# Adamtaranto/mimeo

Hardware: AMD Instinct MI355X
Metric: Gbp-aligned/sec (mimeo self, 1 Gbp genome, --minIdt 80 --minLen 100 --minCov 3) (higher is better)
Workload: dtype int32

## Files before the change

mimeo_amd/csrc/k34_fused.hip:

```cpp
#include <cstdio>
#include <algorithm>
#include <cstdlib>
#include <mutex>
#include <type_traits>

#include "k4_device.h"

namespace mimeo {

constexpr uint32_t TCH = 64;
constexpr uint32_t DQ = 192;
constexpr uint32_t CARE10 = 0x1A997u;
constexpr unsigned long long HEAVY_HITS = 262144;
constexpr unsigned long long PART_HITS = 131072;
constexpr uint32_t HEAVY_GRID = 2048;

struct FusedArgs {
    const FusedUnit *units;
    ExtQueues q;
    HeavyPlan plan;
    int xdrop, hspthresh, transitions;
    uint32_t dbg;
};

struct Bound2 {
    int32_t up, lomax, ub;
    bool stop;
};
template <int W>
__device__ __forceinline__ void bound_block2(Bound2 &B, uint32_t v, uint32_t n, int32_t &lo, int xdrop) {
    const int32_t pv = __popc(v), pn = __popc(n);
    B.ub = max(B.ub, B.up + 100 * W - 100 * pn);
    B.up += 100 * W - 131 * pn - 83 * pv;
    lo += 91 * W - 122 * pn - 94 * pv;
    B.stop = B.stop || (B.up + xdrop < B.lomax);
    B.lomax = max(B.lomax, lo);
}

template <uint32_t CARE, bool TV>
__device__ __forceinline__ uint32_t seed_starts32(uint32_t n0, uint32_t n1, uint32_t d0, uint32_t d1, int transitions) {
    uint32_t ones = 0, twos = 0, tv = 0;
#pragma unroll
    for (int c = 0; c < SEED_LEN; c++) {
        if (!((CARE >> c) & 1u)) continue;
        const uint32_t v = __builtin_amdgcn_alignbit(n1, n0, 13 + c);
        twos |= ones & v;
        ones |= v;
        if (TV) tv |= __builtin_amdgcn_alignbit(d1, d0, 13 + c);
    }
    return ~(transitions ? (twos | tv) : ones);
}

__device__ __forceinline__ bool pair_needs_walk(const uint4 t0, const uint4 t1, const uint4 t2, const uint4 q0, const uint4 q1,
                                                const uint4 q2, int xdrop, int hspthresh, int transitions) {
    const uint32_t dl0 = t0.x ^ q0.x, dl1 = t0.y ^ q0.y, dl2 = t0.z ^ q0.z, dl3 = t0.w ^ q0.w, dl4 = t1.x ^ q1.x, dl5 = t1.y ^ q1.y;
    const uint32_t n0 = dl0 | (t1.z ^ q1.z), n1 = dl1 | (t1.w ^ q1.w), n2 = dl2 | (t2.x ^ q2.x), n3 = dl3 | (t2.y ^ q2.y),
                   n4 = dl4 | (t2.z ^ q2.z), n5 = dl5 | (t2.w ^ q2.w);
    const uint32_t h0 = seed_starts32<CARE10, false>(n2, n3, 0u, 0u, transitions);
    const uint32_t h1 = seed_starts32<CARE10, false>(n1, n2, 0u, 0u, transitions);
    const uint32_t h2 = seed_starts32<CARE10, false>(n0, n1, 0u, 0u, transitions);
    Bound2 L{0, 0, 0, false}, R{0, 0, 0, false};
    int32_t llo = 0, rlo = 0;
    uint32_t veto;
    constexpr uint32_t M24 = 0xFFFFFFu;
    veto = h0 >> 8;
    bound_block2<24>(L, dl3 >> 8, n3 >> 8, llo, xdrop);
    veto |= L.stop ? 0u : ((h0 & 0xFFu) | (h1 >> 16));
    bound_block2<24>(L, __builtin_amdgcn_alignbit(dl3, dl2, 16) & M24, __builtin_amdgcn_alignbit(n3, n2, 16) & M24, llo, xdrop);
    veto |= L.stop ? 0u : ((h1 & 0xFFFFu) | (h2 >> 24));
    bound_block2<24>(L, __builtin_amdgcn_alignbit(dl2, dl1, 24) & M24, __builtin_amdgcn_alignbit(n2, n1, 24) & M24, llo, xdrop);
    veto |= L.stop ? 0u : (h2 & M24);
    bound_block2<24>(L, dl1 & M24, n1 & M24, llo, xdrop);
    bound_block2<24>(R, dl4 & M24, n4 & M24, rlo, xdrop);
    bound_block2<24>(R, __builtin_amdgcn_alignbit(dl5, dl4, 24) & M24, __builtin_amdgcn_alignbit(n5, n4, 24) & M24, rlo, xdrop);
    bound_block2<16>(R, dl5 >> 16, n5 >> 16, rlo, xdrop);
    return !(L.stop && R.stop && L.ub + R.ub < hspthresh && veto == 0);
}

__device__ __forceinline__ bool run_interior(const uint4 t0, const uint4 t1, const uint4 t2, const uint4 q0, const uint4 q1, const uint4 q2,
                                             int transitions) {
    const uint32_t dl3 = t0.w ^ q0.w, dl4 = t1.x ^ q1.x;
    const uint32_t n3 = dl3 | (t2.y ^ q2.y), n4 = dl4 | (t2.z ^ q2.z);
    bool all = true;
#pragma unroll
    for (int k = 0; k < 3; k++) {
        const int off = k == 0 ? 11 : (k == 1 ? 12 : 14);
        const uint32_t wn = __builtin_amdgcn_alignbit(n4, n3, off) & CARE19, wd = __builtin_amdgcn_alignbit(dl4, dl3, off) & CARE19;
        all = all && (transitions ? (wd == 0u && __popc(wn) <= 1) : (wn == 0u));
    }
    return all;
}

constexpr uint32_t DENSE_MIN = 48;
__device__ __forceinline__ uint4 readlane4(const uint4 v, int lane) {
    return make_uint4((uint32_t)__builtin_amdgcn_readlane((int)v.x, lane), (uint32_t)__builtin_amdgcn_readlane((int)v.y, lane),
                      (uint32_t)__builtin_amdgcn_readlane((int)v.z, lane), (uint32_t)__builtin_amdgcn_readlane((int)v.w, lane));
}
__device__ __forceinline__ uint4 bperm4(uint32_t src_lane, const uint4 v) {
    const int a = (int)(src_lane << 2);
    return make_uint4((uint32_t)__builtin_amdgcn_ds_bpermute(a, (int)v.x), (uint32_t)__builtin_amdgcn_ds_bpermute(a, (int)v.y),
                      (uint32_t)__builtin_amdgcn_ds_bpermute(a, (int)v.z), (uint32_t)__builtin_amdgcn_ds_bpermute(a, (int)v.w));
}

template <int THREADS, uint32_t QSEG, bool HEAVY>
struct FusedCfg {
    static constexpr int WAVES = THREADS / 64;
    static constexpr size_t OFF_BYTES = ((TILE_WORDS + 1) * 2 + 15) / 16 * 16;
    static constexpr size_t SMEM = OFF_BYTES + (size_t)QSEG * 48 + (size_t)WAVES * DQ * 4 + (size_t)WAVES * 64 * 8 + QSEG + 16;
};

template <int THREADS, uint32_t QSEG, bool HEAVY>
__global__ __launch_bounds__(THREADS, 4) void k34_scan_extend(FusedArgs A) {
    using Cfg = FusedCfg<THREADS, QSEG, HEAVY>;
    using qoff_t = uint16_t;
    constexpr int WAVES = THREADS / 64;
    static_assert((size_t)QSEG * 48 >= 2 * (TILE_WORDS + 4) * 4, "the count prologue stages both offset arrays in the frame area");
    extern __shared__ __attribute__((aligned(16))) uint8_t smem[];
    qoff_t *sQ = reinterpret_cast<qoff_t *>(smem);
    uint4 *sQF = reinterpret_cast<uint4 *>(smem + Cfg::OFF_BYTES);
    uint32_t *sD_all = reinterpret_cast<uint32_t *>(sQF + QSEG * 3);
    uint2 *s_walk_all = reinterpret_cast<uint2 *>(sD_all + WAVES * DQ);
    uint8_t *sQN = reinterpret_cast<uint8_t *>(s_walk_all + WAVES * 64);
    unsigned long long *s_total = reinterpret_cast<unsigned long long *>(sQN + QSEG);
    __shared__ unsigned long long s_slot;

    const uint32_t lane = threadIdx.x & 63u, wv = threadIdx.x >> 6;
    const uint64_t lt_mask = (1ull << lane) - 1ull;
    uint32_t ai = HEAVY ? 0u : blockIdx.y;
    GFusedUnit U = A.units[ai];
    uint32_t part_p = 0, part_pt = 1, part_qa = 0, part_qb = 0xFFFFFFFFu, part_no = 0;
    uint32_t *sD = sD_all + wv * DQ;
    uint2 *s_walk = s_walk_all + wv * 64;
    uint32_t n_walk = 0;

    auto flush_walk = [&](uint32_t n) {
        __builtin_amdgcn_wave_barrier();
        unsigned long long b = 0;
        const uint32_t shard = (HEAVY ? blockIdx.x + part_no : blockIdx.x) & 7u;
        if (lane == 0) b = atomicAdd(&A.q.nwalk_u[(size_t)ai * 8 + shard], (unsigned long long)n);
        b = __shfl(b, 0);
        if (lane < n && b + lane < U.walk_cap) {
            uint2 e = s_walk[lane];
            e.y = U.Q.pos[e.y] & POS_MASK;
            A.q.walkq[U.walk_base + (size_t)shard * U.walk_cap + b + lane] = e;
        }
        __builtin_amdgcn_wave_barrier();
    };

    auto do_tile = [&](const uint32_t tile) {
        const gptr<uint32_t> toff = U.T.off + (size_t)tile * TILE_WORDS, qoff = U.Q.off + (size_t)tile * TILE_WORDS;
        const uint32_t t0 = toff[0], nT = toff[TILE_WORDS] - t0;
        const uint32_t q0 = qoff[0], nQ = qoff[TILE_WORDS] - q0;
        if (!nT || !nQ) return;
        if (!HEAVY) {
            uint32_t *sT = reinterpret_cast<uint32_t *>(sQF), *sQ32 = sT + TILE_WORDS + 4;
            {
                const gptr<uint4> s0 = toff.as<uint4>(), s1 = qoff.as<uint4>();
                uint4 *d0 = reinterpret_cast<uint4 *>(sT), *d1 = reinterpret_cast<uint4 *>(sQ32);
                for (uint32_t k = threadIdx.x; k < TILE_WORDS / 4; k += THREADS) { const uint4 a = s0[k], b = s1[k]; d0[k] = a; d1[k] = b; }
                if (threadIdx.x == 0) { sT[TILE_WORDS] = t0 + nT; sQ32[TILE_WORDS] = q0 + nQ; *s_total = 0ull; }
            }
            __syncthreads();
            unsigned long long cnt = 0;
            for (uint32_t w = threadIdx.x; w < TILE_WORDS; w += THREADS)
                cnt += (unsigned long long)(sT[w + 1] - sT[w]) * (sQ32[w + 1] - sQ32[w]);
            for (int o = 32; o > 0; o >>= 1) cnt += __shfl_xor(cnt, o);
            if (lane == 0 && cnt) atomicAdd(s_total, cnt);
            __syncthreads();
            if (!*s_total && A.transitions) {
                __syncthreads();
                unsigned long long c2 = 0;
                for (uint32_t w = threadIdx.x; w < TILE_WORDS; w += THREADS) {
                    const uint32_t nt = sT[w + 1] - sT[w];
                    if (nt)
                        for (int j = 0; j < SEED_WEIGHT; j++) { const uint32_t w2 = w ^ (1u << j); c2 += sQ32[w2 + 1] - sQ32[w2]; }
                }
                if (__syncthreads_or(c2 != 0) == 0) return;
            } else if (!*s_total) {
                return;
            }
            const unsigned long long tile_est = *s_total * (A.transitions ? (unsigned long long)(SEED_WEIGHT + 1) : 1ull);
            if (tile_est > HEAVY_HITS || nQ > 0xFFFFu) {
                if (threadIdx.x == 0) {
                    const size_t slot = (size_t)ai * NTILE + atomicAdd(&A.q.nheavy_u[ai], 1ull);
                    A.q.heavy[slot] = tile;
                    A.q.heavy_est[slot] = tile_est;
                }
                return;
            }
        }
        constexpr int NRO = (TILE_WORDS + THREADS) / THREADS;
        uint32_t ro[NRO];
#pragma unroll
        for (int i = 0; i < NRO; i++) {
            const uint32_t k = threadIdx.x + (uint32_t)i * THREADS;
            ro[i] = 0;
            if (k <= TILE_WORDS) ro[i] = (HEAVY ? qoff[k] : (k < TILE_WORDS ? (reinterpret_cast<const uint32_t *>(sQF) + TILE_WORDS + 4)[k] : q0 + nQ)) - q0;
        }
        bool aligned = false;
        uint32_t mid = 0;
        if (!HEAVY && nQ > QSEG) {
            mid = (uint32_t)__builtin_amdgcn_readfirstlane((int)((reinterpret_cast<const uint32_t *>(sQF) + TILE_WORDS + 4)[TILE_WORDS / 2] - q0));
            aligned = mid <= QSEG && nQ - mid <= QSEG;
        }
        const gptr<uint4> tF0 = U.T.fr + t0, tF1 = tF0 + U.T.fr_stride, tF2 = tF1 + U.T.fr_stride;
        const uint32_t nchunks = (nT + TCH - 1) / TCH;
        const uint32_t ch_first = (HEAVY ? part_p * WAVES : 0u) + wv, ch_step = (HEAVY ? part_pt : 1u) * WAVES;
        uint4 nf0 = make_uint4(0, 0, 0, 0), nf1 = nf0, nf2 = nf0;
        uint32_t npos = 0;
        if (ch_first < nchunks) {
            const uint32_t e = ch_first * TCH + lane;
            if (e < nT) { nf0 = tF0[e]; nf1 = tF1[e]; nf2 = tF2[e]; npos = U.T.pos[t0 + e]; }
        }
        unsigned long long hits_acc = 0;
        auto pair_round = [&](const bool valid, const uint4 ta, const uint4 tb, const uint4 tc, const uint32_t tpf, const uint32_t qi, const uint32_t qs) {
            const uint4 qa = sQF[qi], qb = sQF[QSEG + qi], qc = sQF[2 * QSEG + qi];
            const uint32_t qflag = sQN[qi];
            bool need = false;
            uint32_t qp = 0;
            bool live = valid;
            if (HEAVY && !(A.dbg & 16u)) {
                bool inner = false;
                if (valid && ((tpf >> 31) | qflag) == 0 && !U.Tv.svt && run_interior(ta, tb, tc, qa, qb, qc, A.transitions)) {
                    const uint32_t tp = tpf & POS_MASK;
                    inner = tp >= 2u && tp + 1u + SEED_LEN <= U.Tv.len;
                }
                live = valid && !inner;
            }
            if (__ballot(live)) {
                if (live) {
                    if (A.dbg & 1u) need = (ta.x ^ qa.x ^ tb.y ^ qb.y ^ tc.z ^ qc.z) == 0x12345u;
                    else need = ((tpf >> 31) | (qflag & 1u)) != 0 ||
                                pair_needs_walk(ta, tb, tc, qa, qb, qc, A.xdrop, A.hspthresh, A.transitions);
                    if (A.dbg & 2u) need = false;
                }
            }
            if (U.same) {
                if (valid) {
                    qp = U.Q.pos[q0 + qs + qi] & POS_MASK;
                    if ((tpf & POS_MASK) == qp) need = false;
                }
            }
            const uint64_t m = __ballot(need);
            if (m) {
                const uint32_t add = (uint32_t)__popcll(m);
                if (n_walk + add > 64u) { flush_walk(n_walk); n_walk = 0; }
                if (need) s_walk[n_walk + __popcll(m & lt_mask)] = make_uint2(tpf & POS_MASK, q0 + qs + qi);
                n_walk += add;
            }
        };
        const uint32_t q_begin = HEAVY ? part_qa : 0u, q_end = HEAVY ? min(part_qb, nQ) : nQ;
        for (uint32_t qs = q_begin, qe; qs < q_end; qs = qe) {
            qe = aligned ? (qs ? q_end : mid) : min(qs + QSEG, q_end);
            const uint32_t qn = qe - qs;
            const uint32_t half = qs ? 1u : 0u;
            __syncthreads();
#pragma unroll
            for (int i = 0; i < NRO; i++) {
                const uint32_t k = threadIdx.x + (uint32_t)i * THREADS;
                if (k <= TILE_WORDS) sQ[k] = (qoff_t)(min(max(ro[i], qs), qe) - qs);
            }
            {
                const gptr<uint4> s0 = U.Q.fr + q0 + qs, s1 = s0 + U.Q.fr_stride, s2 = s1 + U.Q.fr_stride;
                const gptr<uint32_t> sp = U.Q.pos + q0 + qs;
                for (uint32_t i = threadIdx.x; i < qn; i += THREADS) {
                    const uint4 a = s0[i], b = s1[i], c = s2[i];
                    const uint32_t pq = sp[i], pp = pq & POS_MASK;
                    sQF[i] = a;
                    sQF[QSEG + i] = b;
                    sQF[2 * QSEG + i] = c;
                    sQN[i] = (uint8_t)((pq >> 31) | ((pp >= 2u && pp + 1u + SEED_LEN <= U.Qv.len) ? 0u : 2u));
                }
            }
            __syncthreads();
            for (uint32_t ch = ch_first; ch < nchunks; ch += ch_step) {
                const uint32_t e0 = ch * TCH, ne = min(TCH, nT - e0);
                const uint4 f0 = nf0, f1 = nf1, f2 = nf2;
                const uint32_t mypos = npos;
                {
                    uint32_t nx = ch + ch_step;
                    if (nx >= nchunks) nx = (qe < q_end) ? ch_first : 0xFFFFFFFFu;
                    if (nx != 0xFFFFFFFFu && nx != ch) {
                        const uint32_t e = nx * TCH + lane;
                        if (e < nT) { nf0 = tF0[e]; nf1 = tF1[e]; nf2 = tF2[e]; npos = U.T.pos[t0 + e]; }
                    }
                }
                const bool tvalid = lane < ne;
                uint32_t w = 0, c = 0, nmask = 0, dmask = 0;
                if (tvalid) w = pext12(f2.y >> 13);
                const int nn = A.transitions ? SEED_WEIGHT + 1 : 1;
                if constexpr (!HEAVY) {
                    int jlo = 0, jhi = nn;
                    if (aligned) {
                        const uint64_t in_half = __ballot(tvalid && (w >> 11) == half), in_other = __ballot(tvalid && (w >> 11) != half);
                        if (!in_other) jhi = min(nn, SEED_WEIGHT);
                        else if (!in_half) jlo = SEED_WEIGHT;
                    }
                    jlo = __builtin_amdgcn_readfirstlane(jlo);
                    jhi = __builtin_amdgcn_readfirstlane(jhi);
                    constexpr uint32_t RING = 128;
                    static_assert(RING <= DQ, "the ring lives in the wavefront's descriptor queue");
                    const uint32_t l16 = lane << 16;
                    uint32_t head = 0, tail = 0, pend = 0;
                    uint32_t an = 0, cn = 0;
                    auto fetch = [&](const int jj) {
                        an = 0; cn = 0;
                        if (tvalid && jj < jhi) {
                            const uint32_t w2 = jj ? (w ^ (1u << (jj - 1))) : w;
                            an = sQ[w2];
                            cn = (uint32_t)sQ[w2 + 1] - an;
                        }
                    };
                    auto round = [&](const uint32_t n) {
                        __builtin_amdgcn_wave_barrier();
                        const bool valid = lane < n;
                        const uint32_t d = valid ? sD[(head + lane) & (RING - 1u)] : 0u;
                        const uint32_t owner = d >> 16, qi = d & 0xFFFFu;
                        if (!(A.dbg & 4u)) {
                            const uint4 ta = bperm4(owner, f0), tb = bperm4(owner, f1), tc = bperm4(owner, f2);
                            const uint32_t tpf = (uint32_t)__builtin_amdgcn_ds_bpermute((int)(owner << 2), (int)mypos);
                            pair_round(valid, ta, tb, tc, tpf, qi, qs);
                        }
                        __builtin_amdgcn_wave_barrier();
                        head = (head + 64u) & (RING - 1u);
                        pend -= n;
                    };
                    fetch(jlo);
#pragma unroll 1
                    for (int j = jlo; j < jhi; j++) {
                        const uint32_t ak = l16 | an, cnt = cn;
                        fetch(j + 1);
                        uint32_t k = 0;
#pragma unroll 1
                        for (uint64_t m = __ballot(cnt > 0u); m; m = __ballot(cnt > k)) {
                            if (cnt > k) {
                                const uint32_t slot = __builtin_amdgcn_mbcnt_hi((uint32_t)(m >> 32), __builtin_amdgcn_mbcnt_lo((uint32_t)m, tail));
                                sD[slot & (RING - 1u)] = ak + k;
                            }
                            const uint32_t add = (uint32_t)__popcll(m);
                            tail = (tail + add) & (RING - 1u);
                            pend += add;
                            hits_acc += add;
                            k++;
                            if (pend >= 64u) round(64u);
                        }
                    }
                    if (pend) round(pend);
                } else {
                    auto probes = [&]() {
                        if (!tvalid) return;
                        for (int j = 0; j < nn; j++) {
                            const uint32_t w2 = j ? (w ^ (1u << (j - 1))) : w;
                            const uint32_t a = sQ[w2], b = sQ[w2 + 1];
                            if (b - a >= DENSE_MIN) { dmask |= 1u << j; continue; }
                            c += b - a;
                            nmask |= (b != a ? 1u : 0u) << j;
                        }
                    };
                    probes();
                    uint32_t inc = c;
                    inc += (uint32_t)__builtin_amdgcn_update_dpp(0, (int)inc, 0x111, 0xf, 0xf, false);
                    inc += (uint32_t)__builtin_amdgcn_update_dpp(0, (int)inc, 0x112, 0xf, 0xf, false);
                    inc += (uint32_t)__builtin_amdgcn_update_dpp(0, (int)inc, 0x114, 0xf, 0xf, false);
                    inc += (uint32_t)__builtin_amdgcn_update_dpp(0, (int)inc, 0x118, 0xf, 0xf, false);
                    inc += (uint32_t)__builtin_amdgcn_update_dpp(0, (int)inc, 0x142, 0xa, 0xf, false);
                    inc += (uint32_t)__builtin_amdgcn_update_dpp(0, (int)inc, 0x143, 0xc, 0xf, false);
                    const uint32_t tot = (uint32_t)__builtin_amdgcn_readlane((int)inc, 63), st = inc - c;
                    hits_acc += tot;
                    for (uint32_t rb = 0; rb < tot; rb += DQ) {
                        if (!(A.dbg & 8u) && c && st < rb + DQ && st + c > rb) {
                            uint32_t acc = st;
                            const uint32_t wend = rb + DQ;
                            for (uint32_t m = nmask; m; m &= m - 1u) {
                                const uint32_t j = (uint32_t)__builtin_ctz(m);
                                const uint32_t w2 = j ? (w ^ (1u << (j - 1u))) : w;
                                const uint32_t a = sQ[w2], cnt = (uint32_t)sQ[w2 + 1] - a, d0 = (lane << 16) | a;
                                if (acc >= rb && acc + cnt <= wend) {
                                    uint32_t *dst = sD + (acc - rb);
                                    dst[0] = d0;
                                    if (cnt > 1) {
                                        dst[1] = d0 + 1u;
#pragma unroll 1
                                        for (uint32_t k = 2; k < cnt; k++) dst[k] = d0 + k;
                                    }
                                } else {
                                    const uint32_t g0 = max(acc, rb), g1 = min(acc + cnt, wend);
#pragma unroll 1
                                    for (uint32_t g = g0; g < g1; g++) sD[g - rb] = d0 + (g - acc);
                                }
                                acc += cnt;
                            }
                        }
                        __builtin_amdgcn_wave_barrier();
                        const uint32_t n = (A.dbg & 4u) ? 0u : min(DQ, tot - rb);
                        for (uint32_t i = 0; i < n; i += 64) {
                            const bool valid = i + lane < n;
                            const uint32_t d = valid ? sD[i + lane] : 0u;
                            const uint32_t owner = d >> 16, qi = d & 0xFFFFu;
                            const uint4 ta = bperm4(owner, f0), tb = bperm4(owner, f1), tc = bperm4(owner, f2);
                            const uint32_t tpf = (uint32_t)__builtin_amdgcn_ds_bpermute((int)(owner << 2), (int)mypos);
                            pair_round(valid, ta, tb, tc, tpf, qi, qs);
                        }
                        __builtin_amdgcn_wave_barrier();
                    }
                    for (uint64_t lm = __ballot(dmask != 0u); lm; lm &= lm - 1ull) {
                        const int o = __builtin_ctzll(lm);
                        const uint4 ta = readlane4(f0, o), tb = readlane4(f1, o), tc = readlane4(f2, o);
                        const uint32_t tpf = (uint32_t)__builtin_amdgcn_readlane((int)mypos, o), wo = (uint32_t)__builtin_amdgcn_readlane((int)w, o);
                        for (uint32_t dm = (uint32_t)__builtin_amdgcn_readlane((int)dmask, o); dm; dm &= dm - 1u) {
                            const uint32_t j = (uint32_t)__builtin_ctz(dm), w2 = j ? (wo ^ (1u << (j - 1u))) : wo;
                            const uint32_t a = sQ[w2], b = sQ[w2 + 1];
                            hits_acc += b - a;
                            if (A.dbg & 4u) continue;
                            for (uint32_t i = a; i < b; i += 64u) {
                                const bool valid = i + lane < b;
                                pair_round(valid, ta, tb, tc, tpf, valid ? i + lane : a, qs);
                            }
                        }
                    }
                }
            }
        }
        if (lane == 0 && hits_acc) atomicAdd(&A.q.tile_hits[(size_t)U.unit * NTILE + tile], hits_acc);
    };

    if (!HEAVY) {
        do_tile(blockIdx.x);
    } else {
        __shared__ uint32_t s_part;
        const uint32_t nparts = A.plan.ctr[2], ntiles = A.plan.ctr[1];
        for (;;) {
            __syncthreads();
            if (threadIdx.x == 0) s_part = atomicAdd(&A.plan.ctr[0], 1u);
            __syncthreads();
            const uint32_t g = s_part;
            if (g >= nparts) break;
            uint32_t lo = 0, hi = ntiles;
            while (hi - lo > 1) {
                const uint32_t mid = (lo + hi) >> 1;
                if (A.plan.base[mid] <= g) lo = mid; else hi = mid;
            }
            const uint2 ut = A.plan.tile[lo];
            const uint4 sp = A.plan.split[lo];
            const uint32_t part = g - A.plan.base[lo];
            if (n_walk && ut.x != ai) { flush_walk(n_walk); n_walk = 0; }
            ai = ut.x;
            U = A.units[ai];
            part_no = part;
            part_p = part % sp.x; part_pt = sp.x;
            part_qa = (part / sp.x) * sp.z; part_qb = part_qa + sp.z;
            do_tile(ut.y);
        }
    }
    if (n_walk) flush_walk(n_walk);
    (void)s_slot;
}

__global__ __launch_bounds__(256) void k34_sum_hits(const unsigned long long *__restrict__ tile_hits, unsigned long long *__restrict__ unit_hits) {
    __shared__ unsigned long long red[256];
    unsigned long long s = 0;
    for (uint32_t i = threadIdx.x; i < NTILE; i += 256) s += tile_hits[(size_t)blockIdx.x * NTILE + i];
    red[threadIdx.x] = s;
    __syncthreads();
    for (int o = 128; o > 0; o >>= 1) {
        if ((int)threadIdx.x < o) red[threadIdx.x] += red[threadIdx.x + o];
        __syncthreads();
    }
    if (threadIdx.x == 0) unit_hits[blockIdx.x] = red[0];
}
void launch_sum_hits(const ExtQueues &q, uint32_t nunits, hipStream_t st) {
    hipLaunchKernelGGL(k34_sum_hits, dim3(nunits), dim3(256), 0, st, (const unsigned long long *)q.tile_hits, q.unit_hits);
}

__global__ __launch_bounds__(1024) void k34_plan(const FusedUnit *__restrict__ units, uint32_t nunits, ExtQueues q, HeavyPlan P) {
    __shared__ uint32_t s_scan[1024];
    __shared__ uint32_t s_carry, s_tiles;
    const uint32_t tid = threadIdx.x;
    if (tid == 0) { s_carry = 0; s_tiles = 0; }
    __syncthreads();
    for (uint32_t u = 0; u < nunits; u++) {
        const uint32_t nlist = (uint32_t)min((unsigned long long)NTILE, q.nheavy_u[u]);
        const GFusedUnit U = units[u];
        for (uint32_t i0 = 0; i0 < nlist; i0 += 1024) {
            const uint32_t i = i0 + tid;
            uint32_t parts = 0, pt = 1, pq = 1, qlen = 0, tile = 0;
            if (i < nlist) {
                tile = q.heavy[(size_t)u * NTILE + i];
                const unsigned long long est = P.est[(size_t)u * NTILE + i];
                const gptr<uint32_t> toff = U.T.off + (size_t)tile * TILE_WORDS, qoff = U.Q.off + (size_t)tile * TILE_WORDS;
                const uint32_t nT = toff[TILE_WORDS] - toff[0], nQ = qoff[TILE_WORDS] - qoff[0];
                const uint32_t want = (uint32_t)min((unsigned long long)(1u << 20), (est + PART_HITS - 1) / PART_HITS);
                const uint32_t groups = max(1u, (nT + 511u) / 512u);
                pt = min(groups, max(1u, want));
                const uint32_t need_q = max(1u, (want + pt - 1) / pt);
                qlen = max(64u, (((nQ + need_q - 1) / need_q) + 63u) & ~63u);
                pq = max(1u, (nQ + qlen - 1) / qlen);
                parts = pt * pq;
            }
            s_scan[tid] = parts;
            __syncthreads();
            for (uint32_t o = 1; o < 1024; o <<= 1) {
                const uint32_t v = tid >= o ? s_scan[tid - o] : 0u;
                __syncthreads();
                s_scan[tid] += v;
                __syncthreads();
            }
            if (i < nlist) {
                const uint32_t k = s_tiles + (i - i0);
                P.tile[k] = make_uint2(u, tile);
                P.split[k] = make_uint4(pt, pq, qlen, 0u);
                P.base[k] = s_carry + s_scan[tid] - parts;
            }
            __syncthreads();
            if (tid == 1023) { s_carry += s_scan[1023]; s_tiles += min(1024u, nlist - i0); }
            __syncthreads();
        }
    }
    if (tid == 0) { P.base[s_tiles] = s_carry; P.ctr[0] = 0; P.ctr[1] = s_tiles; P.ctr[2] = s_carry; }
}

constexpr uint32_t QSEG_FIRST = 1280, QSEG_HEAVY = 1024;

int launch_fused_batch(const FusedUnit *d_units, uint32_t nactive, const ExtQueues &q, const HeavyPlan &plan, const mimeo_params *p, hipStream_t st,
                       uint32_t dbg) {
    if (!nactive) return 0;
    FusedArgs A;
    A.units = d_units; A.q = q;
    A.xdrop = p->xdrop; A.hspthresh = p->hspthresh; A.transitions = p->transitions;
    A.dbg = dbg;
    constexpr size_t smem_heavy = FusedCfg<512, QSEG_HEAVY, true>::SMEM, smem_first = FusedCfg<512, QSEG_FIRST, false>::SMEM;
    static std::once_flag attr_once;
    static hipError_t attr_err = hipSuccess;
    std::call_once(attr_once, [&] {
        attr_err = hipFuncSetAttribute(reinterpret_cast<const void *>(k34_scan_extend<512, QSEG_FIRST, false>),
                                       hipFuncAttributeMaxDynamicSharedMemorySize, (int)smem_first);
        if (attr_err == hipSuccess)
            attr_err = hipFuncSetAttribute(reinterpret_cast<const void *>(k34_scan_extend<512, QSEG_HEAVY, true>),
                                           hipFuncAttributeMaxDynamicSharedMemorySize, (int)smem_heavy);
    });
    HIP_TRY(attr_err);
    for (uint32_t u0 = 0; u0 < nactive; u0 += 32768u) {
        const uint32_t nu = std::min(32768u, nactive - u0);
        FusedArgs B = A;
        B.units = d_units + u0;
        B.q.nwalk_u = q.nwalk_u + (size_t)u0 * 8; B.q.nheavy_u = q.nheavy_u + u0; B.q.heavy = q.heavy + (size_t)u0 * NTILE;
        B.q.heavy_est = q.heavy_est + (size_t)u0 * NTILE;
        B.plan = plan;
        B.plan.est = B.q.heavy_est;
        hipLaunchKernelGGL((k34_scan_extend<512, QSEG_FIRST, false>), dim3(NTILE, nu), dim3(512), smem_first, st, B);
        hipLaunchKernelGGL(k34_plan, dim3(1), dim3(1024), 0, st, B.units, nu, B.q, B.plan);
        hipLaunchKernelGGL((k34_scan_extend<512, QSEG_HEAVY, true>), dim3(HEAVY_GRID), dim3(512), smem_heavy, st, B);
    }
    return 0;
}

}
```

mimeo_amd/csrc/k4_device.h:

```cpp
#pragma once
#include "device_util.h"

namespace mimeo {

constexpr uint32_t CARE19 = 0x7A997u;
constexpr int EXT_THREADS = 256;
constexpr int LONG_WINDOWS = 8;

struct ExtCounters {
    unsigned long long ncand, nfollow, nlong, nhsp, nmed, nbig, nwalked;
    unsigned long long nfollow8[8], nmed8[8];
    unsigned long long nbigcand;
    unsigned long long long_next, seg_next;
    unsigned long long nwalk_total, nwalk_over;
    unsigned long long dbg[8];
};

struct HeavyPlan {
    const unsigned long long *est;
    uint2 *tile;
    uint32_t *base;
    uint4 *split;
    unsigned int *ctr;
};
struct Cand {
    uint32_t tstart, qstart, len;
    int32_t raw;
    uint32_t unit;
};
constexpr int32_t RAW_SATURATED = 0x7FFFFFFF;

struct ExtQueues {
    ExtCounters *ctr;
    Cand *cand;
    uint64_t *fkey;
    uint32_t *fprev;
    uint2 *medq, *longq;
    uint32_t *medu, *longu;
    uint2 *walkq;
    unsigned long long *nwalk_u;
    unsigned long long *nheavy_u;
    uint32_t *heavy;
    unsigned long long *heavy_est;
    unsigned long long *bigcand;
    unsigned long long *bigacc;
    unsigned long long *unit_hits;
    unsigned long long *tile_hits;
    uint64_t cand_cap, follow_cap, med_cap, long_cap, walk_cap;
    uint32_t ebits, dbits;
};
__device__ __forceinline__ uint32_t queue_shard() { return blockIdx.x & 7u; }
__device__ __forceinline__ unsigned long long wave_slot(unsigned long long *counter) {
    const uint64_t m = __ballot(true);
    const uint32_t lane = threadIdx.x & 63u, lead = (uint32_t)__builtin_ctzll(m);
    unsigned long long b = 0;
    if (lane == lead) b = atomicAdd(counter, (unsigned long long)__popcll(m));
    b = __shfl(b, (int)lead);
    return b + __popcll(m & ((1ull << lane) - 1ull));
}
__device__ __forceinline__ uint64_t follow_key(const ExtQueues &q, uint32_t unit, int32_t d, uint32_t qlen, uint32_t et) {
    return ((uint64_t)unit << (q.dbits + q.ebits)) | ((uint64_t)(uint32_t)(d + (int32_t)qlen) << q.ebits) | (uint64_t)et;
}
__device__ __forceinline__ uint32_t key_unit(const ExtQueues &q, uint64_t k) { return (uint32_t)(k >> (q.dbits + q.ebits)); }
__device__ __forceinline__ uint32_t key_end(const ExtQueues &q, uint64_t k) { return (uint32_t)(k & ((1ull << q.ebits) - 1ull)); }
__device__ __forceinline__ uint64_t key_unit_diag(const ExtQueues &q, uint64_t k) { return k >> q.ebits; }
__device__ __forceinline__ int32_t key_diag(const ExtQueues &q, uint64_t k, uint32_t qlen) {
    return (int32_t)(uint32_t)((k >> q.ebits) & ((1ull << q.dbits) - 1ull)) - (int32_t)qlen;
}

constexpr uint32_t RUN_END = 0xFFFFFFFFu;

__device__ __forceinline__ bool seed_hit_at(const GStrandView &T, const GStrandView &Q, int32_t p, int32_t d,
                                            int transitions) {
    int32_t pq = p - d;
    const Win32 tw = win32(T, p), qw = win32(Q, pq);
    if (!((seedvalid32(T, p, tw.sv) & qw.sv) & 1u)) return false;
    uint32_t dl = (tw.lo ^ qw.lo) & CARE19;
    uint32_t dh = (tw.hi ^ qw.hi) & CARE19;
    if (!transitions) return (dl | dh) == 0;
    return dl == 0 && __popc(dh) <= 1;
}

constexpr int GROUP_TAB = 4096;
constexpr int QCAP = 64;
constexpr int FAST_THREADS = 512;

static inline int host_sub(int dl, int dh, int cg) {
    static const int lo[4] = {91, 100, -31, -31}, hi[4] = {-114, -114, -123, -125};
    return (dl ? hi : lo)[(dh << 1) | cg];
}
static inline void build_group_table(uint32_t *tab) {
    for (int idx = 0; idx < GROUP_TAB; idx++) {
        int p = 0, M = -100000, mn = 100000, posM = 0;
        for (int k = 0; k < 4; k++) {
            p += host_sub((idx >> k) & 1, (idx >> (4 + k)) & 1, (idx >> (8 + k)) & 1);
            if (p > M) { M = p; posM = k; }
            if (p < mn) mn = p;
        }
        tab[idx] = ((uint32_t)p & 0x3FFu) | (((uint32_t)M & 0x3FFu) << 10) | (((uint32_t)mn & 0x3FFu) << 20) |
                   ((uint32_t)posM << 30);
    }
}

struct WalkState {
    int32_t run, best;
    uint32_t bk, k;
    bool done, found;
    uint32_t found_step;
};

template <int G = 4>
__device__ __forceinline__ void walk_window(const uint32_t *__restrict__ tab, WalkState &w, uint32_t mdl, uint32_t mdh,
                                            uint32_t mcg, uint32_t mnn, uint32_t mH, uint32_t limit, int xdrop,
                                            uint32_t start = 0) {
    constexpr uint32_t GM = (1u << G) - 1u;
    for (uint32_t pos = start; pos < 32;) {
        const uint32_t rem = limit - w.k;
        if (rem == 0) { w.done = true; return; }
        if (rem >= (uint32_t)G && pos <= 32u - G && !(((mnn | mH) >> pos) & GM)) {
            const uint32_t idx = ((mdl >> pos) & GM) | (((mdh >> pos) & GM) << G) | (((mcg >> pos) & GM) << (2 * G));
            const uint32_t e = tab[idx];
            const int32_t S = ((int32_t)(e << 22)) >> 22, M = ((int32_t)(e << 12)) >> 22, mn = ((int32_t)(e << 2)) >> 22;
            if (w.run + mn < w.best - xdrop) { w.done = true; return; }
            if (w.run + M > w.best) { w.best = w.run + M; w.bk = w.k + (e >> 30) + 1; }
            w.run += S;
            w.k += G;
            pos += G;
        } else {
            w.k++;
            w.run += sub_score((mdl >> pos) & 1u, (mdh >> pos) & 1u, (mcg >> pos) & 1u, (mnn >> pos) & 1u);
            if (w.run > w.best) { w.best = w.run; w.bk = w.k; }
            if (w.run < w.best - xdrop) { w.done = true; return; }
            if ((mH >> pos) & 1u) { w.found = true; w.found_step = w.k; w.done = true; return; }
            pos++;
        }
    }
}

template <int G = 4>
__device__ __forceinline__ void walk_window_pred(const uint32_t *__restrict__ tab, WalkState &w, uint32_t mdl,
                                                 uint32_t mdh, uint32_t mcg, uint32_t mnn, uint32_t mH, uint32_t limit,
                                                 int xdrop) {
    constexpr uint32_t GM = (1u << G) - 1u;
    constexpr int NG = 32 / G, LOG = G == 4 ? 2 : 1;
    static_assert(G == 4 || G == 2, "group size");
    const uint32_t blocked = mnn | mH;
    uint32_t ent[NG];
#pragma unroll
    for (int c = 0; c < NG; c++) {
        const int pos = G * c;
        ent[c] = tab[((mdl >> pos) & GM) | (((mdh >> pos) & GM) << G) | (((mcg >> pos) & GM) << (2 * G))];
    }
    uint32_t nz = blocked | (blocked >> 1);
    if (G == 4) nz |= nz >> 2;
    const uint32_t ng = (limit - w.k) >> LOG;
    nz |= ng >= (uint32_t)NG ? 0u : (0xFFFFFFFFu << ((uint32_t)G * ng));
    int32_t R = w.run, B = w.best, sR = R, sB = B;
    uint32_t BK = 0, sBK = 0, sC = 0;
    bool stopped = w.done, slow = false, brkdone = false;
#pragma unroll
    for (int c = 0; c < NG; c++) {
        const uint32_t e = ent[c];
        const int32_t S = ((int32_t)(e << 22)) >> 22, M = ((int32_t)(e << 12)) >> 22, mn = ((int32_t)(e << 2)) >> 22;
        const bool blk = (nz >> (G * c)) & 1u;
        const bool brk = R + mn + xdrop < B;
        const bool first = (blk || brk) && !stopped;
        sR = first ? R : sR;
        sB = first ? B : sB;
        sBK = first ? BK : sBK;
        sC = first ? (uint32_t)c : sC;
        slow = slow || (first && blk);
        brkdone = brkdone || (first && !blk);
        stopped = stopped || blk || brk;
        const int32_t cand = R + M;
        BK = cand > B ? (e >> 30) + (uint32_t)(G * c + 1) : BK;
        B = max(B, cand);
        R += S;
    }
    if (!stopped) { sR = R; sB = B; sBK = BK; sC = NG; }
    w.run = sR;
    w.best = sB;
    w.bk = sBK ? w.k + sBK : w.bk;
    w.k += (uint32_t)G * sC;
    w.done = w.done || brkdone;
    if (__ballot(slow)) {
        if (slow) walk_window<G>(tab, w, mdl, mdh, mcg, mnn, mH, limit, xdrop, (uint32_t)G * sC);
    }
}

template <int G>
__device__ __forceinline__ uint32_t group_table_entry(uint32_t idx) {
    int32_t p = 0, M = -100000, mn = 100000, posM = 0;
#pragma unroll
    for (int k = 0; k < G; k++) {
        p += sub_score((idx >> k) & 1u, (idx >> (G + k)) & 1u, (idx >> (2 * G + k)) & 1u, 0u);
        if (p > M) { M = p; posM = k; }
        if (p < mn) mn = p;
    }
    return ((uint32_t)p & 0x3FFu) | (((uint32_t)M & 0x3FFu) << 10) | (((uint32_t)mn & 0x3FFu) << 20) | ((uint32_t)posM << 30);
}

__device__ __forceinline__ uint32_t ext32(uint32_t a, uint32_t b, uint32_t c, uint32_t sh) {
    return sh < 32 ? __builtin_amdgcn_alignbit(b, a, sh) : __builtin_amdgcn_alignbit(c, b, sh - 32);
// ... 593 lines not shown
```

mimeo_amd/csrc/k4_extend.hip:

```cpp
#include <algorithm>
#include <cmath>
#include <cstdio>
#include <cstdlib>
#include <cstring>
#include <mutex>
#include <utility>

#include <rocprim/rocprim.hpp>

#include "k4_device.h"

namespace mimeo {

__global__ __launch_bounds__(EXT_THREADS) void k4_extend_generic(const UnitDesc *__restrict__ units, ExtQueues q, int xdrop,
                                                              int hspthresh, int transitions,
                                                              const uint32_t *__restrict__ group_tab) {
    __shared__ uint32_t tab[GROUP_TAB];
    for (int i = threadIdx.x; i < GROUP_TAB; i += EXT_THREADS) tab[i] = group_tab[i];
    __syncthreads();
    uint64_t sh_end[8];
    {
        uint64_t acc = 0;
#pragma unroll
        for (int r = 0; r < 8; r++) { acc += min((uint64_t)q.ctr->nmed8[r], q.med_cap); sh_end[r] = acc; }
// ... 29 lines not shown
    auto flush_cd = [&]() {
        __builtin_amdgcn_wave_barrier();
        unsigned long long b = 0;
        if (lane == 0) b = atomicAdd(&q.ctr->ncand, (unsigned long long)n_cd);
        b = __shfl(b, 0) + lane;
        if (lane < n_cd && b < q.cand_cap) q.cand[b] = s_cd[wv][lane];
        n_cd = 0;
        __builtin_amdgcn_wave_barrier();
    };
    const uint64_t stride = (uint64_t)gridDim.x * EXT_THREADS;
    for (uint64_t g0 = (uint64_t)blockIdx.x * EXT_THREADS + wv * 64u; g0 < nhits; g0 += stride) {
        const uint64_t gid = g0 + lane;
        bool o_fol = false, o_long = false, o_cd = false;
        uint64_t r_fk = 0;
        uint32_t r_fp = 0, unit = 0;
        uint2 h = make_uint2(0, 0);
        Cand r_cd{0, 0, 0, 0, 0};
        if (gid < nhits) {
            uint32_t r = 0;
#pragma unroll
            for (int k = 0; k < 7; k++) r += gid >= sh_end[k] ? 1u : 0u;
            const uint64_t at = (uint64_t)r * q.med_cap + (gid - (r ? sh_end[r - 1] : 0));
            h = q.medq[at];
            unit = q.medu[at];
            const GStrandView T = units[unit].T, Q = units[unit].Q;
            const int32_t et = (int32_t)h.x + SEED_LEN, eq = (int32_t)h.y + SEED_LEN;
            const int32_t d = (int32_t)h.x - (int32_t)h.y;
            WalkState L{0, 0, 0, 0, false, false, 0};
            const uint32_t maxl = (uint32_t)min(et, eq);
            bool is_long = false;
            for (int win = 0; !L.done; win++) {
                if (win == LONG_WINDOWS) { is_long = true; break; }
                const int32_t P = et - 32 * (win + 1) - SEED_LEN, Pq = P - d;
                const Win64 tw = win64(T, P), qw = win64(Q, Pq);
                const uint64_t dl64 = tw.lo ^ qw.lo, dh64 = tw.hi ^ qw.hi, nm64 = dl64 | dh64;
                const uint32_t nlo = (uint32_t)nm64, nhi = (uint32_t)(nm64 >> 32);
                const uint32_t tlo = (uint32_t)dl64, thi = (uint32_t)(dl64 >> 32);
                uint32_t ones = 0, twos = 0, tv = 0;
#pragma unroll
                for (int c = 0; c < SEED_LEN; c++) {
                    if (!((CARE19 >> c) & 1u)) continue;
                    const uint32_t v = c ? __builtin_amdgcn_alignbit(nhi, nlo, c) : nlo;
                    twos |= ones & v;
                    ones |= v;
                    tv |= c ? __builtin_amdgcn_alignbit(thi, tlo, c) : tlo;
                }
                const uint32_t bad = transitions ? (twos | tv) : ones;
                const uint32_t H = ~bad & seedvalid32(T, P, (uint32_t)tw.sv) & (uint32_t)qw.sv;
                walk_window(tab, L, __brev((uint32_t)(dl64 >> SEED_LEN)), __brev((uint32_t)(dh64 >> SEED_LEN)),
                            __brev((uint32_t)((tw.lo ^ tw.hi) >> SEED_LEN)), __brev((uint32_t)((tw.nm | qw.nm) >> SEED_LEN)),
                            __brev(H), maxl, xdrop);
            }
            if (!is_long && L.found) {
                o_fol = true;
                r_fk = follow_key(q, unit, d, Q.len, (uint32_t)et);
                r_fp = (uint32_t)et - L.found_step;
            } else {
                WalkState R{0, 0, 0, 0, false, false, 0};
                if (!is_long) {
                    const uint32_t maxr = min(T.len - (uint32_t)et, Q.len - (uint32_t)eq);
                    for (int win = 0; !R.done; win++) {
                        if (win == LONG_WINDOWS) { is_long = true; break; }
                        const int32_t P = et + 32 * win, Pq = P - d;
                        const Win32 tw = win32(T, P), qw = win32(Q, Pq);
                        walk_window(tab, R, tw.lo ^ qw.lo, tw.hi ^ qw.hi, tw.lo ^ tw.hi, tw.nm | qw.nm, 0u, maxr, xdrop);
                    }
                }
                if (is_long) o_long = true;
                else {
                    const int32_t score = L.best + R.best;
                    if (score >= hspthresh) { o_cd = true; r_cd = Cand{(uint32_t)et - L.bk, (uint32_t)eq - L.bk, L.bk + R.bk, score, unit}; }
                }
            }
        }
        uint64_t m = __ballot(o_fol);
        if (m) {
            const uint32_t add = (uint32_t)__popcll(m);
            if (n_fol + add > GCAP) flush_fol();
            if (o_fol) { const uint32_t i = n_fol + (uint32_t)__popcll(m & lt_mask); s_fk[wv][i] = r_fk; s_fp[wv][i] = r_fp; }
            n_fol += add;
        }
        m = __ballot(o_long);
        if (m) {
            const uint32_t add = (uint32_t)__popcll(m);
            if (n_long + add > GCAP) flush_long();
            if (o_long) { const uint32_t i = n_long + (uint32_t)__popcll(m & lt_mask); s_lh[wv][i] = h; s_lu[wv][i] = unit; }
            n_long += add;
        }
        m = __ballot(o_cd);
        if (m) {
            const uint32_t add = (uint32_t)__popcll(m);
            if (n_cd + add > GCAP) flush_cd();
            if (o_cd) s_cd[wv][n_cd + (uint32_t)__popcll(m & lt_mask)] = r_cd;
            n_cd += add;
        }
    }
    if (n_fol) flush_fol();
    if (n_long) flush_long();
    if (n_cd) flush_cd();
}

template <int VARIANT>
__device__ __forceinline__ void extend_hits_body(const GStrandView &T, const GStrandView &Q,
                                                 const uint2 *__restrict__ hits, uint64_t nhits,
                                                 int xdrop, int hspthresh, int transitions,
                                                 const uint32_t *__restrict__ group_tab, const ExtQueues &q, uint32_t unit,
                                                 int skip_diag0, const unsigned long long *__restrict__ nhits_dev) {
    constexpr bool FILTER = VARIANT == 5 || VARIANT == 9;
    constexpr int SCAP = 256;
    uint64_t sh_end[8] = {0, 0, 0, 0, 0, 0, 0, 0};
    const uint64_t shard_cap = nhits;
    if (nhits_dev) {
        uint64_t acc = 0;
#pragma unroll
        for (int r = 0; r < 8; r++) { acc += min((uint64_t)nhits_dev[r], shard_cap); sh_end[r] = acc; }
        nhits = acc;
    }
    __shared__ uint32_t tab[GROUP_TAB];
    __shared__ uint2 s_med[FAST_THREADS / 64][SCAP];
    __shared__ uint64_t s_fk[FAST_THREADS / 64][SCAP];
    __shared__ uint32_t s_fp[FAST_THREADS / 64][SCAP];
    __shared__ Cand s_cd[FAST_THREADS / 64][QCAP];
    __shared__ uint2 s_walk[FILTER ? FAST_THREADS / 64 : 1][QCAP];
    for (int i = threadIdx.x; i < GROUP_TAB; i += FAST_THREADS) tab[i] = group_tab[i];
    __syncthreads();
    const uint32_t lane = threadIdx.x & 63u, wv = threadIdx.x >> 6;
    const uint64_t lt_mask = (1ull << lane) - 1ull;
    WaveFill fill{0, 0, 0};
    uint32_t n_walk = 0, n_walked = 0;

    auto walk_batch = [&](bool active, uint2 h, bool final) {
        bool q_med = false, q_fol = false, q_cd = false;
        uint64_t r_fk = 0;
        uint32_t r_fp = 0;
        Cand r_cd{0, 0, 0, 0, 0};
        if (active) walk_hit<1>(tab, T, Q, h, xdrop, hspthresh, transitions, q_med, q_fol, q_cd, r_fk, r_fp, r_cd);
        stage_records<true, SCAP>(q, unit, s_med[wv], s_fk[wv], s_fp[wv], s_cd[wv], fill, q_med, h, q_fol, r_fk, r_fp, q_cd, r_cd, final);
    };

    const uint64_t stride = (uint64_t)gridDim.x * FAST_THREADS;
    for (uint64_t g0 = (uint64_t)blockIdx.x * FAST_THREADS + wv * 64u; g0 < nhits; g0 += stride) {
        const uint64_t gid = g0 + lane;
        uint2 h = make_uint2(0, 0);
        if (gid < nhits) {
            uint64_t at = gid;
            if (nhits_dev) {
                uint32_t r = 0;
#pragma unroll
                for (int k = 0; k < 7; k++) r += gid >= sh_end[k] ? 1u : 0u;
                at = (uint64_t)r * shard_cap + (gid - (r ? sh_end[r - 1] : 0));
            }
            h = hits[at];
        }
        const bool valid = gid < nhits && !(skip_diag0 && h.x == h.y);
        if (!FILTER) {
            walk_batch(valid, h, false);
        } else {
            bool need = false;
            if (valid)
                need = VARIANT == 9 ? hit_needs_walk<16, true>(T, Q, h, xdrop, hspthresh, transitions)
                                    : hit_needs_walk<16, false>(T, Q, h, xdrop, hspthresh, transitions);
            const uint64_t m = __ballot(need);
            if (m) {
                const uint32_t add = (uint32_t)__popcll(m);
                if (n_walk + add > (uint32_t)QCAP) {
                    __builtin_amdgcn_wave_barrier();
                    const uint2 hq = s_walk[wv][lane < n_walk ? lane : 0];
                    walk_batch(lane < n_walk, hq, false);
                    n_walked += n_walk;
                    n_walk = 0;
                    __builtin_amdgcn_wave_barrier();
                }
                if (need) s_walk[wv][n_walk + __popcll(m & lt_mask)] = h;
                n_walk += add;
            }
        }
    }
    if (FILTER && n_walk) {
        __builtin_amdgcn_wave_barrier();
        const uint2 hq = s_walk[wv][lane < n_walk ? lane : 0];
        walk_batch(lane < n_walk, hq, false);
        n_walked += n_walk;
    }
    __shared__ unsigned int s_nwalked;
    if (FILTER) {
        if (threadIdx.x == 0) s_nwalked = 0;
        __syncthreads();
        if (n_walked && lane == 0) atomicAdd(&s_nwalked, n_walked);
        __syncthreads();
        if (threadIdx.x == 0 && s_nwalked) atomicAdd(&q.ctr->nwalked, (unsigned long long)s_nwalked);
    }
    walk_batch(false, make_uint2(0, 0), true);
    if (!nhits_dev && blockIdx.x == 0 && threadIdx.x == 0) q.unit_hits[unit] = nhits;
}
template <int VARIANT>
__global__ __launch_bounds__(FAST_THREADS) void k4_extend_hits(StrandView T, StrandView Q, const uint2 *__restrict__ hits, uint64_t nhits,
                                                              int xdrop, int hspthresh, int transitions,
                                                              const uint32_t *__restrict__ group_tab, ExtQueues q, uint32_t unit, int skip_diag0) {
    extend_hits_body<VARIANT>(T, Q, hits, nhits, xdrop, hspthresh, transitions, group_tab, q, unit, skip_diag0, nullptr);
}
template <int VARIANT>
__global__ __launch_bounds__(FAST_THREADS) void k4_walk_batch(const FusedUnit *__restrict__ funits, int xdrop, int hspthresh, int transitions,
                                                             const uint32_t *__restrict__ group_tab, ExtQueues q) {
    const FusedUnit &U = funits[blockIdx.y];
    const GStrandView T = U.Tv, Q = U.Qv;
    extend_hits_body<VARIANT>(T, Q, q.walkq + U.walk_base, U.walk_cap, xdrop, hspthresh, transitions, group_tab, q, U.unit, 0,
                              q.nwalk_u + (size_t)blockIdx.y * 8);
}

__global__ __launch_bounds__(256) void k4_walk_summary(const FusedUnit *__restrict__ funits, uint32_t nactive, const unsigned long long *__restrict__ nwalk_u,
                                                       ExtCounters *ctr) {
    unsigned long long tot = 0, worst = 0;
    for (uint32_t i = blockIdx.x * 256 + threadIdx.x; i < nactive * 8u; i += gridDim.x * 256) {
        const unsigned long long n = nwalk_u[i], cap = funits[i >> 3].walk_cap;
        tot += n;
        worst = max(worst, cap ? (n * 1024ull + cap - 1) / cap : (n ? 1ull << 40 : 0ull));
    }
    for (int o = 32; o > 0; o >>= 1) { tot += __shfl_xor(tot, o); worst = max(worst, (unsigned long long)__shfl_xor(worst, o)); }
    if ((threadIdx.x & 63) == 0) { if (tot) atomicAdd(&ctr->nwalk_total, tot); if (worst) atomicMax(&ctr->nwalk_over, worst); }
}

constexpr uint32_t CLAIM = 16;
__global__ __launch_bounds__(EXT_THREADS) void k4_extend_long(const UnitDesc *__restrict__ units, ExtQueues q, int xdrop,
                                                              int hspthresh, int transitions) {
    __shared__ WaveStage s_stage[EXT_THREADS / 64];
    WaveStage &S = s_stage[threadIdx.x >> 6];
    uint32_t nf = 0, nc = 0;
    const uint64_t nlong = min((uint64_t)q.ctr->nlong, q.long_cap);
    for (;;) {
        unsigned long long w0 = 0;
        if ((threadIdx.x & 63u) == 0) w0 = atomicAdd(&q.ctr->long_next, (unsigned long long)CLAIM);
        w0 = ((unsigned long long)(uint32_t)__builtin_amdgcn_readfirstlane((int)(uint32_t)(w0 >> 32)) << 32) | (uint32_t)__builtin_amdgcn_readfirstlane((int)(uint32_t)w0);
        if (w0 >= nlong) break;
        for (uint64_t wid = w0; wid < min(nlong, (uint64_t)w0 + CLAIM); wid++) {
            const uint32_t unit = q.longu[wid];
            stage_push(S, nf, nc, wave_extend_record(units[unit].T, units[unit].Q, q.longq[wid], xdrop, hspthresh, transitions, true, q, unit, nullptr), q);
        }
    }
    stage_flush(S, nf, nc, q);
}

__global__ __launch_bounds__(256) void k4_compact_followers(ExtQueues q, uint64_t *__restrict__ key, uint32_t *__restrict__ prev) {
    uint64_t sh_end[8];
    uint64_t acc = 0;
#pragma unroll
    for (int r = 0; r < 8; r++) { acc += min((uint64_t)q.ctr->nfollow8[r], q.follow_cap); sh_end[r] = acc; }
    if (blockIdx.x == 0 && threadIdx.x == 0) q.ctr->nfollow = acc;
    for (uint64_t gid = (uint64_t)blockIdx.x * 256 + threadIdx.x; gid < acc; gid += (uint64_t)gridDim.x * 256) {
        uint32_t r = 0;
#pragma unroll
        for (int k = 0; k < 7; k++) r += gid >= sh_end[k] ? 1u : 0u;
        const uint64_t at = (uint64_t)r * q.follow_cap + (gid - (r ? sh_end[r - 1] : 0));
        key[gid] = q.fkey[at];
        prev[gid] = q.fprev[at];
    }
}

__global__ void k4_segment_flags(const uint64_t *__restrict__ key, const uint32_t *__restrict__ prev, uint64_t n,
                                 ExtQueues q, uint8_t *__restrict__ flag) {
    uint64_t i = (uint64_t)blockIdx.x * blockDim.x + threadIdx.x;
    if (i >= n) return;
    bool start = true;
    if (i > 0) {
        uint64_t a = key[i - 1], b = key[i];
        start = prev[i] != RUN_END && (key_unit_diag(q, a) != key_unit_diag(q, b) || key_end(q, a) != prev[i]);
    }
    flag[i] = start ? 1 : 0;
}

constexpr uint32_t SMALL_SEG = 8;
__global__ __launch_bounds__(EXT_THREADS) void k4_resolve_small(const UnitDesc *__restrict__ units, ExtQueues q,
                                                                const uint64_t *__restrict__ key,
                                                                const uint32_t *__restrict__ prev, uint64_t nfollow,
                                                                const uint64_t *__restrict__ seg_start,
                                                                const uint64_t *__restrict__ nseg_dev,
                                                                int xdrop, int hspthresh,
                                                                const uint32_t *__restrict__ group_tab,
                                                                uint64_t *__restrict__ bigseg) {
    __shared__ uint32_t tab[GROUP_TAB];
    const uint64_t nseg = *nseg_dev;
    if ((uint64_t)blockIdx.x * EXT_THREADS >= nseg) return;
    for (int i = threadIdx.x; i < GROUP_TAB; i += EXT_THREADS) tab[i] = group_tab[i];
    __syncthreads();
    const uint64_t sid = (uint64_t)blockIdx.x * EXT_THREADS + threadIdx.x;
    if (sid >= nseg) return;
    const uint64_t beg = seg_start[sid], end = sid + 1 < nseg ? seg_start[sid + 1] : nfollow;
    bool big = end - beg > SMALL_SEG;
    Cand out[SMALL_SEG];
    uint32_t nout = 0;
    const uint32_t unit = key_unit(q, key[beg]);
    if (!big) {
        const GStrandView T = units[unit].T, Q = units[unit].Q;
        const int32_t d = key_diag(q, key[beg], Q.len);
        const int32_t het = (int32_t)prev[beg];
        WalkState H{0, 0, 0, 0, false, false, 0};
        big = !lane_walk(tab, T, Q, het, d, +1, min(T.len - (uint32_t)het, Q.len - (uint32_t)(het - d)), xdrop, H);
        uint32_t reach = (uint32_t)het + H.bk;
        for (uint64_t i = beg; i < end && !big; i++) {
            const uint32_t hi = key_end(q, key[i]);
            const uint32_t lo = prev[i] == RUN_END ? key_end(q, key[i - 1]) + 1u : hi;
            for (uint32_t et = max(lo, reach + 1u); et <= hi && !big; et = reach + 1u) {
                const int32_t eq = (int32_t)et - d;
                WalkState L{0, 0, 0, 0, false, false, 0}, R{0, 0, 0, 0, false, false, 0};
                if (nout == SMALL_SEG ||
                    !lane_walk(tab, T, Q, (int32_t)et, d, -1, (uint32_t)min((int32_t)et, eq), xdrop, L) ||
                    !lane_walk(tab, T, Q, (int32_t)et, d, +1, min(T.len - et, Q.len - (uint32_t)eq), xdrop, R)) {
                    big = true;
                    break;
                }
                if (L.best + R.best >= hspthresh) out[nout++] = Cand{et - L.bk, (uint32_t)eq - L.bk, L.bk + R.bk, L.best + R.best, unit};
                reach = et + R.bk;
            }
        }
    }
// ... 798 lines not shown
```

Before: 0.04432.

## Apply sharp walk filter at fused-kernel flush and skip re-filtering marked hits

In the non-heavy fused seed kernel, walk candidates are re-checked at flush time with a sharper window filter that loads the target and query fragments again from global memory. Only survivors are enqueued, compacted with a ballot, and tagged with a high-bit flag. The extend kernel then skips its own hit_needs_walk filter for tagged hits. The intent is fewer queued walks and no repeated filtering, at the cost of extra global loads and arithmetic inside the fused kernel and a dependence on positions never using the flag bit.

```diff
diff --git a/mimeo_amd/csrc/k34_fused.hip b/mimeo_amd/csrc/k34_fused.hip
--- a/mimeo_amd/csrc/k34_fused.hip
+++ b/mimeo_amd/csrc/k34_fused.hip
@@ -77,6 +77,25 @@
     return !(L.stop && R.stop && L.ub + R.ub < hspthresh && veto == 0);
 }
 
+__device__ __forceinline__ bool pair_needs_walk_sharp(const uint4 t0, const uint4 t1, const uint4 t2, const uint4 q0, const uint4 q1,
+                                                      const uint4 q2, int xdrop, int hspthresh, int transitions) {
+    const uint32_t dl0 = t0.x ^ q0.x, dl1 = t0.y ^ q0.y, dl2 = t0.z ^ q0.z, dl3 = t0.w ^ q0.w, dl4 = t1.x ^ q1.x, dl5 = t1.y ^ q1.y;
+    const uint32_t dh0 = t1.z ^ q1.z, dh1 = t1.w ^ q1.w, dh2 = t2.x ^ q2.x, dh3 = t2.y ^ q2.y, dh4 = t2.z ^ q2.z, dh5 = t2.w ^ q2.w;
+    const uint32_t n0 = dl0 | dh0, n1 = dl1 | dh1, n2 = dl2 | dh2, n3 = dl3 | dh3;
+    const uint32_t h0 = seed_starts32<CARE19, true>(n2, n3, dl2, dl3, transitions);
+    const uint32_t h1 = seed_starts32<CARE19, true>(n1, n2, dl1, dl2, transitions);
+    const uint32_t h2 = seed_starts32<CARE19, true>(n0, n1, dl0, dl1, transitions) & 0xFFFF0000u;
+    Bound L{0, 0, 0, 0, false}, R{0, 0, 0, 0, false};
+    bound_window<16, true>(L, dl3, dh3, t0.w ^ t2.y, xdrop);
+    bound_window<16, true>(L, dl2, dh2, t0.z ^ t2.x, xdrop);
+    const bool stop64 = L.stop;
+    bound_window<16, true, 1>(L, dl1, dh1, t0.y ^ t1.w, xdrop);
+    bound_window<16, false>(R, dl4, dh4, t1.x ^ t2.z, xdrop);
+    bound_window<16, false>(R, dl5, dh5, t1.y ^ t2.w, xdrop);
+    const uint32_t veto = h0 | h1 | (stop64 ? 0u : h2);
+    return !(L.stop && R.stop && L.ub + R.ub < hspthresh && veto == 0);
+}
+
 __device__ __forceinline__ bool run_interior(const uint4 t0, const uint4 t1, const uint4 t2, const uint4 q0, const uint4 q1, const uint4 q2,
                                              int transitions) {
     const uint32_t dl3 = t0.w ^ q0.w, dl4 = t1.x ^ q1.x;
@@ -135,14 +154,27 @@
 
     auto flush_walk = [&](uint32_t n) {
         __builtin_amdgcn_wave_barrier();
-        unsigned long long b = 0;
         const uint32_t shard = (HEAVY ? blockIdx.x + part_no : blockIdx.x) & 7u;
-        if (lane == 0) b = atomicAdd(&A.q.nwalk_u[(size_t)ai * 8 + shard], (unsigned long long)n);
-        b = __shfl(b, 0);
-        if (lane < n && b + lane < U.walk_cap) {
-            uint2 e = s_walk[lane];
-            e.y = U.Q.pos[e.y] & POS_MASK;
-            A.q.walkq[U.walk_base + (size_t)shard * U.walk_cap + b + lane] = e;
+        uint2 e = make_uint2(0, 0);
+        bool keep = lane < n;
+        if (keep) {
+            const uint2 s = s_walk[lane];
+            const uint32_t tp = U.T.pos[s.x], qp = U.Q.pos[s.y];
+            e = make_uint2(tp & POS_MASK, qp & POS_MASK);
+            if (!HEAVY && !(A.dbg & 32u)) {
+                const gptr<uint4> tf = U.T.fr + s.x, qf = U.Q.fr + s.y;
+                const uint4 ta = tf[0], tb = tf[U.T.fr_stride], tc = tf[2 * (size_t)U.T.fr_stride];
+                const uint4 qa = qf[0], qb = qf[U.Q.fr_stride], qc = qf[2 * (size_t)U.Q.fr_stride];
+                keep = ((tp | qp) & POS_NFLAG) != 0 || pair_needs_walk_sharp(ta, tb, tc, qa, qb, qc, A.xdrop, A.hspthresh, A.transitions);
+                e.x |= WALK_SHARP_DONE;
+            }
+        }
+        const uint64_t km = __ballot(keep);
+        if (km) {
+            unsigned long long b = 0;
+            if (lane == 0) b = atomicAdd(&A.q.nwalk_u[(size_t)ai * 8 + shard], (unsigned long long)__popcll(km));
+            b = __shfl(b, 0) + __popcll(km & lt_mask);
+            if (keep && b < U.walk_cap) A.q.walkq[U.walk_base + (size_t)shard * U.walk_cap + b] = e;
         }
         __builtin_amdgcn_wave_barrier();
     };
@@ -213,7 +245,7 @@
             if (e < nT) { nf0 = tF0[e]; nf1 = tF1[e]; nf2 = tF2[e]; npos = U.T.pos[t0 + e]; }
         }
         unsigned long long hits_acc = 0;
-        auto pair_round = [&](const bool valid, const uint4 ta, const uint4 tb, const uint4 tc, const uint32_t tpf, const uint32_t qi, const uint32_t qs) {
+        auto pair_round = [&](const bool valid, const uint4 ta, const uint4 tb, const uint4 tc, const uint32_t tpf, const uint32_t te, const uint32_t qi, const uint32_t qs) {
             const uint4 qa = sQF[qi], qb = sQF[QSEG + qi], qc = sQF[2 * QSEG + qi];
             const uint32_t qflag = sQN[qi];
             bool need = false;
@@ -245,7 +277,7 @@
             if (m) {
                 const uint32_t add = (uint32_t)__popcll(m);
                 if (n_walk + add > 64u) { flush_walk(n_walk); n_walk = 0; }
-                if (need) s_walk[n_walk + __popcll(m & lt_mask)] = make_uint2(tpf & POS_MASK, q0 + qs + qi);
+                if (need) s_walk[n_walk + __popcll(m & lt_mask)] = make_uint2(te, q0 + qs + qi);
                 n_walk += add;
             }
         };
@@ -319,7 +351,7 @@
                         if (!(A.dbg & 4u)) {
                             const uint4 ta = bperm4(owner, f0), tb = bperm4(owner, f1), tc = bperm4(owner, f2);
                             const uint32_t tpf = (uint32_t)__builtin_amdgcn_ds_bpermute((int)(owner << 2), (int)mypos);
-                            pair_round(valid, ta, tb, tc, tpf, qi, qs);
+                            pair_round(valid, ta, tb, tc, tpf, t0 + e0 + owner, qi, qs);
                         }
                         __builtin_amdgcn_wave_barrier();
                         head = (head + 64u) & (RING - 1u);
@@ -399,7 +431,7 @@
                             const uint32_t owner = d >> 16, qi = d & 0xFFFFu;
                             const uint4 ta = bperm4(owner, f0), tb = bperm4(owner, f1), tc = bperm4(owner, f2);
                             const uint32_t tpf = (uint32_t)__builtin_amdgcn_ds_bpermute((int)(owner << 2), (int)mypos);
-                            pair_round(valid, ta, tb, tc, tpf, qi, qs);
+                            pair_round(valid, ta, tb, tc, tpf, t0 + e0 + owner, qi, qs);
                         }
                         __builtin_amdgcn_wave_barrier();
                     }
@@ -414,7 +446,7 @@
                             if (A.dbg & 4u) continue;
                             for (uint32_t i = a; i < b; i += 64u) {
                                 const bool valid = i + lane < b;
-                                pair_round(valid, ta, tb, tc, tpf, valid ? i + lane : a, qs);
+                                pair_round(valid, ta, tb, tc, tpf, t0 + e0 + (uint32_t)o, valid ? i + lane : a, qs);
                             }
                         }
                     }
diff --git a/mimeo_amd/csrc/k4_device.h b/mimeo_amd/csrc/k4_device.h
--- a/mimeo_amd/csrc/k4_device.h
+++ b/mimeo_amd/csrc/k4_device.h
@@ -49,6 +49,7 @@
     uint64_t cand_cap, follow_cap, med_cap, long_cap, walk_cap;
     uint32_t ebits, dbits;
 };
+constexpr uint32_t WALK_SHARP_DONE = 0x80000000u;
 __device__ __forceinline__ uint32_t queue_shard() { return blockIdx.x & 7u; }
 __device__ __forceinline__ unsigned long long wave_slot(unsigned long long *counter) {
     const uint64_t m = __ballot(true);
diff --git a/mimeo_amd/csrc/k4_extend.hip b/mimeo_amd/csrc/k4_extend.hip
--- a/mimeo_amd/csrc/k4_extend.hip
+++ b/mimeo_amd/csrc/k4_extend.hip
@@ -205,14 +205,18 @@
             }
             h = hits[at];
         }
+        const bool marked = nhits_dev && (h.x & WALK_SHARP_DONE) != 0;
+        if (nhits_dev) h.x &= POS_MASK;
         const bool valid = gid < nhits && !(skip_diag0 && h.x == h.y);
         if (!FILTER) {
             walk_batch(valid, h, false);
         } else {
-            bool need = false;
-            if (valid)
-                need = VARIANT == 9 ? hit_needs_walk<16, true>(T, Q, h, xdrop, hspthresh, transitions)
-                                    : hit_needs_walk<16, false>(T, Q, h, xdrop, hspthresh, transitions);
+            bool need = valid && marked;
+            if (__ballot(valid && !marked)) {
+                if (valid && !marked)
+                    need = VARIANT == 9 ? hit_needs_walk<16, true>(T, Q, h, xdrop, hspthresh, transitions)
+                                        : hit_needs_walk<16, false>(T, Q, h, xdrop, hspthresh, transitions);
+            }
             const uint64_t m = __ballot(need);
             if (m) {
                 const uint32_t add = (uint32_t)__popcll(m);
```

New measurement: 0.04570 (median of 6 runs). 1.03x the previous value.
